# LeiXu84/fireFoam-dev

Measured on AMD Instinct MI355X. Metric: PIMPLE outer-iterations/sec on 64M-cell hex mesh; pEqn SpMV GB/s vs HBM peak, higher is better.
Workload: dtype f64; 1 GPU; synthetic 400^3 hex box (64000000 cells), buoyant plume + 5-species EDC-shaped source, PIMPLE 1/2/0: rhoEqn + UEqn + YEEqn(4 Yi + h) + 2 pEqn per step; cells=64000000, faces=191520000, parallelism=1 GPU, transport_solvers=PBiCGStab+DILU

## Files before the change

### firefoam-dev_amd/binding.py

```python
import ctypes as C
import os
import re
import subprocess

import numpy as np

_HERE = os.path.dirname(os.path.abspath(__file__))
_ROOT = os.path.dirname(_HERE)
_SO = os.path.join(_HERE, "lib", "libffm.so")
_HDR = os.path.join(_ROOT, "include", "ffm.h")

SOLVERS = {"PCG": 0, "PBiCGStab": 1, "PBiCG": 2, "diagonal": 3, "smoothSolver": 4}
PRECONDS = {"none": 0, "DIC": 1, "DILU": 2, "GaussSeidel": 3, "symGaussSeidel": 4, "diagonal": 5}


class FfmError(RuntimeError):
    pass


class Perf(C.Structure):
    _fields_ = [("initialResidual", C.c_double), ("finalResidual", C.c_double),
                ("nIterations", C.c_int), ("converged", C.c_int), ("singular", C.c_int)]

    def as_dict(self):
# ... 65 lines not shown
        "ffm_ldu_set_coeffs_d": ([vp, dp, dp, dp], C.c_int),
        "ffm_ldu_n_native_faces": ([vp], C.c_int),
        "ffm_ldu_get_face_map": ([vp, ip], C.c_int),
        "ffm_ldu_set_coeffs_native_d": ([vp, dp, dp, dp], C.c_int),
        "ffm_ldu_bind_coeffs_native_d": ([vp, dp, dp, dp, C.c_int], C.c_int),
        "ffm_ldu_set_interfaces": ([vp, C.c_int, ip, C.POINTER(ip), C.POINTER(hp), C.POINTER(hp), ip], C.c_int),
        "ffm_ldu_set_global_cells": ([vp, C.c_long], C.c_int),
        "ffm_spmv": ([vp, dp, dp], C.c_int),
        "ffm_tmul": ([vp, dp, dp], C.c_int),
        "ffm_sumA": ([vp, dp], C.c_int),
        "ffm_residual": ([vp, dp, dp, dp], C.c_int),
        "ffm_precond_setup": ([vp, C.c_int, dp], C.c_int),
        "ffm_precond_apply": ([vp, C.c_int, C.c_int, dp, dp], C.c_int),
        "ffm_precond_setup_multi": ([vp, C.c_int, C.c_int, C.POINTER(C.c_void_p), C.POINTER(C.c_void_p)], C.c_int),
        "ffm_ldu_tile_reach": ([vp, C.POINTER(C.c_int), C.POINTER(C.c_int), C.POINTER(C.c_int)], C.c_int),
        "ffm_gs_smooth": ([vp, C.c_int, C.c_int, dp, dp], C.c_int),
        "ffm_solve_d": ([vp, C.c_int, C.c_int, C.c_double, C.c_double, C.c_int, C.c_int, C.c_int, dp, dp,
                         C.POINTER(Perf)], C.c_int),
        "ffm_solve": ([vp, C.c_int, C.c_int, C.c_double, C.c_double, C.c_int, C.c_int, C.c_int, hp, hp,
                       C.POINTER(Perf)], C.c_int),
        "ffm_solve_multi_d": ([vp, C.c_int, C.c_int, C.c_int, C.c_double, C.c_double, C.c_int, C.c_int, C.POINTER(C.c_void_p), dp, dp,
                               C.POINTER(C.c_void_p), C.POINTER(C.c_void_p), C.POINTER(Perf)], C.c_int),
        "ffm_ldu_unbind_coeffs": ([vp], C.c_int),
        "ffm_ldu_offdiag_epoch": ([vp], C.c_ulong),
        "ffm_ldu_tile_coef_read": ([vp, C.c_int, hp], C.c_int),
        "ffm_ldu_tile_gathers": ([vp], C.c_long),
        "ffm_debug_pool_poison": ([vp, C.c_int], C.c_int),
        "ffm_bench_spmv": ([vp, dp, dp, C.c_int, hp], C.c_int),
        "ffm_bench_precond": ([vp, C.c_int, dp, dp, C.c_int, hp], C.c_int),
        "ffm_debug_set_sweep_ticket": ([vp, C.c_uint], C.c_int),
# ... 80 lines not shown
                                           + [C.POINTER(C.c_void_p)] * 16, C.c_int),
        "ffm_fvm_scalar_transport_multi_w": ([vp, C.c_int, dp, C.c_double, dp, dp, dp, dp, dp, dp] + [C.POINTER(C.c_void_p)] * 12, C.c_int),
        "ffm_fvm_scalar_transport_multi_ws": ([vp, C.c_int, dp, C.c_double, dp, dp, dp, dp, dp, dp] + [C.POINTER(C.c_void_p)] * 5 + [hp]
                                              + [C.POINTER(C.c_void_p)] * 7, C.c_int),
        "ffm_fvm_scalar_transport_multi_ws_direct": ([vp, C.c_int, dp, C.c_double, dp, dp, dp, dp, dp, dp] + [C.POINTER(C.c_void_p)] * 5 + [hp]
                                                     + [C.POINTER(C.c_void_p)] * 7, C.c_int),
        "ffm_fv_multivariate_weights": ([vp, C.c_int, C.POINTER(C.c_int), C.c_double, C.c_double, C.c_double, dp] + [C.POINTER(C.c_void_p)] * 4 + [dp], C.c_int),
        "ffm_fvm_lust_source3": ([vp, C.c_double, dp, dp] + [C.POINTER(C.c_void_p)] * 5, C.c_int),
        "ffm_pc_phig": ([vp, dp, dp, dp, dp], C.c_int),
        "ffm_ue_buoyancy_flux": ([vp, dp, dp, dp, dp], C.c_int),
        "ffm_pc_phiHbyA": ([vp, dp, dp, dp, dp, dp, dp, dp, dp], C.c_int),
        "ffm_pc_flux": ([vp, dp, dp, dp, dp, dp, dp, dp, dp, dp], C.c_int),
        "ffm_pc_face_fluxes": ([vp] + [dp] * 10, C.c_int),
        "ffm_pc_finish": ([vp, C.c_double, C.c_double] + [dp] * 9 + [C.POINTER(vp)] + [dp] * 4 + [C.POINTER(vp)] + [dp] * 4, C.c_int),
        "ffm_ue_buoyancy_source3": ([vp, dp, dp, dp, dp, C.POINTER(vp), C.POINTER(vp), dp, C.POINTER(vp), C.POINTER(vp), C.POINTER(vp)], C.c_int),
        "ffm_fvm_transport_scheme": ([vp, C.c_double, dp, dp, C.c_int, dp, C.c_int, dp, dp, dp], C.c_int),
        "ffm_fvm_transport_scheme_direct": ([vp, C.c_double, dp, dp, C.c_int, dp, C.c_int, dp, dp, dp], C.c_int),
        "ffm_fvc_div_dev2T_gradU": ([vp, C.POINTER(vp), dp, dp, C.POINTER(vp), C.POINTER(vp), C.POINTER(vp)], C.c_int),
        "ffm_les_keqn_G": ([vp, C.POINTER(vp), dp, dp], C.c_int),
        "ffm_fvm_HbyA3": ([vp, dp, dp, C.POINTER(vp), C.POINTER(vp), C.POINTER(vp), C.POINTER(vp), dp, C.POINTER(vp)], C.c_int),
        "ffm_fvc_flux_rho": ([vp, dp, dp, dp, dp, dp], C.c_int),
        "ffm_fvm_pressure_eqn": ([vp, C.c_double] + [dp] * 6 + [C.c_double] + [dp] * 9, C.c_int),
        "ffm_fvm_pressure_eqn_direct": ([vp, C.c_double] + [dp] * 6 + [C.c_double] + [dp] * 9, C.c_int),
        "ffm_fvc_ddt_corr": ([vp, C.c_double] + [dp] * 6, C.c_int),
        "ffm_fvc_rho_eqn": ([vp, C.c_double] + [dp] * 4, C.c_int),
        "ffm_fvc_div_phiK_terms": ([vp, C.c_int] + [C.c_double] * 4 + [dp] * 14, C.c_int),
        "ffm_fvdom_ray_assemble_d": ([vp, hp] + [C.c_double] * 3 + [dp] * 9, C.c_int),
        "ffm_fvdom_wall_coeffs_d": ([vp, C.c_int, C.c_int, hp, hp, C.c_double] + [dp] * 8, C.c_int),
        "ffm_fvdom_sum_rays_d": ([vp, C.c_int, dp, dp], C.c_int),
        "ffm_mesh_nboundary": ([vp], C.c_int),
# ... 476 lines not shown

    def reciprocalD_multi(self, preconditioner, diags):
        self.ctx._ready()
        n = len(diags)
        out = [self.ctx.empty(self.nCells) for _ in range(n)]
        arr = lambda ts: (C.c_void_p * n)(*[t.data_ptr() for t in ts])
        _check(lib().ffm_precond_setup_multi(self.h, PRECONDS[preconditioner], n, arr(diags), arr(out)), "ffm_precond_setup_multi")
        self.ctx.sync()
        return out

    def tile_reach(self):
        r, a, b = C.c_int(), C.c_int(), C.c_int()
        _check(lib().ffm_ldu_tile_reach(self.h, C.byref(r), C.byref(a), C.byref(b)), "ffm_ldu_tile_reach")
        return r.value, a.value, b.value

    def precondition(self, preconditioner, rA, transpose=False):
        self.ctx._ready()
        w = self.ctx.empty(self.nCells)
        _check(lib().ffm_precond_apply(self.h, PRECONDS[preconditioner], 1 if transpose else 0,
                                       C.c_void_p(rA.data_ptr()), C.c_void_p(w.data_ptr())), "ffm_precond_apply")
        self.ctx.sync()
        return w

    def smooth(self, psi, source, nSweeps=1, smoother="symGaussSeidel"):
        self.ctx._ready()
        psi = psi.clone()
        self.ctx._ready()
        _check(lib().ffm_gs_smooth(self.h, 1 if smoother == "symGaussSeidel" else 0, nSweeps,
                                   C.c_void_p(psi.data_ptr()), C.c_void_p(source.data_ptr())), "ffm_gs_smooth")
        self.ctx.sync()
# ... 471 lines not shown
```

### firefoam-dev_amd/csrc/ffm_device.hpp

```cpp
#pragma once
#include <hip/hip_runtime.h>
#include "ffm_internal.hpp"

static inline int sgrid(long n) { long g = (n + 255) / 256; return (int)std::max(1L, std::min(g, (long)RED_BLOCKS)); }

__device__ __forceinline__ double wave_sum(double v)
{
#pragma unroll
    for (int o = 32; o > 0; o >>= 1) v += __shfl_down(v, o, 64);
    return v;
}
__device__ __forceinline__ double wave_min(double v)
{
#pragma unroll
    for (int o = 32; o > 0; o >>= 1) v = fmin(v, __shfl_down(v, o, 64));
    return v;
}
__device__ __forceinline__ double wave_max(double v)
{
#pragma unroll
    for (int o = 32; o > 0; o >>= 1) v = fmax(v, __shfl_down(v, o, 64));
    return v;
}

// ... 115 lines not shown
__device__ __forceinline__ void load_lower(const LduView &v, int c, RowEnt<W> &R, int s0 = 0)
{
    const int sl = c >> 6, lane = c & 63;
    const int lb = lo_base(v, sl) + s0 * 64, lw = lo_width(v, sl) - s0;
    int e[W];
#pragma unroll
    for (int s = 0; s < W; s++) e[s] = (s < lw) ? (NT ? __builtin_nontemporal_load(&v.loEnt[lb + s * 64 + lane]) : v.loEnt[lb + s * 64 + lane]) : -1;
#pragma unroll
    for (int s = 0; s < W; s++) {
        R.on[s] = e[s] >= 0;
        R.nb[s] = R.on[s] ? (e[s] >> v.loShift) : c;
        R.f[s] = R.on[s] ? face_of(v, R.nb[s], (int)__builtin_amdgcn_ubfe((unsigned)e[s], 0u, (unsigned)v.loShift)) : 0;
    }
}

template <int W, bool MASK_GHOST = false, bool NT = false>
__device__ __forceinline__ void load_upper(const LduView &v, int c, RowEnt<W> &R, int s0 = 0)
{
    const int sl = c >> 6, lane = c & 63;
    const int ub = up_base(v, sl) + s0 * 64, uw = up_width(v, sl) - s0;
#pragma unroll
    for (int s = 0; s < W; s++) {
        const int idx = ub + s * 64 + lane;
        const int n = (s < uw) ? (NT ? __builtin_nontemporal_load(&v.upNbr[idx]) : v.upNbr[idx]) : -1;
        R.on[s] = n >= 0 && (!MASK_GHOST || n < v.N);
        R.nb[s] = R.on[s] ? n : c;
        R.f[s] = R.on[s] ? idx : 0;
    }
}

// ... 21 lines not shown
```

### firefoam-dev_amd/csrc/ffm_fused.hip

```cpp
#include "ffm_mesh.hpp"

constexpr int FUSE_MAX = 5;
constexpr int FUSE_MAX_OWN = 4;
#define CHECK_M(m) if (!(m)) { ffm_set_error("null mesh"); return FFM_ERR_ARG; }

struct GradMulti {
    const double *vf[FUSE_MAX], *vb[FUSE_MAX];
    double *gx[FUSE_MAX], *gy[FUSE_MAX], *gz[FUSE_MAX];
};

template <int W, int NF>
__global__ __launch_bounds__(256) void k_grad_multi(MeshView q, GradMulti a)
{
    CELL_SCHED(ci, q) {
        const int c = (int)ci;
        RowEnt<W> L, U; load_lower<W>(q.v, c, L); load_upper<W>(q.v, c, U);
        double wl[W], wu[W], sx[2 * W], sy[2 * W], sz[2 * W];
#pragma unroll
        for (int s = 0; s < W; s++) {
            wl[s] = q.w[L.f[s]]; wu[s] = q.w[U.f[s]];
            sx[s] = q.Sfx[L.f[s]]; sy[s] = q.Sfy[L.f[s]]; sz[s] = q.Sfz[L.f[s]];
            sx[W + s] = q.Sfx[U.f[s]]; sy[W + s] = q.Sfy[U.f[s]]; sz[W + s] = q.Sfz[U.f[s]];
        }
        const double V = q.V[c];
// ... 1009 lines not shown
    if (!ghf || !rho || !p_rgh || !diag || !source || !diagOut || !sourceOut || (m->B && (!t_b || !ic || !bc))) return FFM_ERR_ARG;
    UeBuoyancy a;
    for (int d = 0; d < 3; d++) {
        if (!source[d] || !diagOut[d] || !sourceOut[d] || (m->B && (!ic[d] || !bc[d]))) return FFM_ERR_ARG;
        a.ic[d] = m->B ? ic[d] : nullptr; a.bc[d] = m->B ? bc[d] : nullptr; a.src[d] = source[d]; a.diagOut[d] = diagOut[d]; a.srcOut[d] = sourceOut[d];
    }
    a.ghf = ghf; a.rho = rho; a.prgh = p_rgh; a.tb = t_b; a.diag = diag; a.invT = m->invT; a.bMagSf = m->bMagSf; a.invStride = m->N;
    if (m->A->maxW > 8) return FFM_ERR_UNSUPPORTED;
    if (m->A->maxW <= 3) LAUNCH_CELLS(k_ue_buoyancy_source3<3>, mview(m), a);
    else if (m->A->maxW <= 4) LAUNCH_CELLS(k_ue_buoyancy_source3<4>, mview(m), a);
    else LAUNCH_CELLS(k_ue_buoyancy_source3<8>, mview(m), a);
    FFM_HIP(hipGetLastError());
    return FFM_OK;
}

struct PEqn {
    const double *psi, *psi0, *p0, *rho, *rho0, *gh, *gamma, *phiHbyA, *phiHbyAb, *ic, *bc;
    double *upper, *lower, *diag, *src;
    double rdt, pRef;
    TileCoefOut tile;
};
template <int W, bool TILE = false>
__global__ __launch_bounds__(256, (TILE ? 8 : 1)) void k_p_rgh_eqn(MeshView q, PEqn a)
{
    CELL_SCHED(ci, q) {
        const int c = (int)ci;
        RowEnt<W> L, U; load_lower<W>(q.v, c, L); load_upper<W>(q.v, c, U);
        double dLap = 0.0, acc = 0.0;
        double vl[TILE ? W : 1] = {}, vu[TILE ? W : 1] = {};
#pragma unroll
// ... 298 lines not shown
```

### firefoam-dev_amd/csrc/ffm_plume_step.hip

```cpp
#include "ffm_plume.hpp"

static void bc_update_f(ffm_plume *P, double *f, const double *fStatic)
{ const double *pb = P->phib; forN(P, P->B, [=] __device__(long k) { f[k] = fStatic[k] < 0 ? 1.0 - (pb[k] >= 0 ? 1.0 : 0.0) : fStatic[k]; }); }

static int update_bcs(ffm_plume *P)
{
    for (int c = 0; c < 3; c++) bc_update_f(P, P->fU[c], P->fStaticU[c]);
    bc_update_f(P, P->fS, P->fStaticS);
    bc_update_f(P, P->fH, P->fStaticH);
    return FFM_OK;
}

static int U_boundary(ffm_plume *P)
{
    for (int c = 0; c < 3; c++) FFM_TRY(ffm_bc_values(P->mesh, P->fU[c], P->refU[c], P->zeroB, P->U[c], P->Ub[c]));
    return FFM_OK;
}

static int bc_p_rgh(ffm_plume *P, const double *grad , const double *rhob)
{
    const double *kind = P->kind_d, *pb = P->phib, *phb = P->ph_rgh_b;
    const double *u0 = P->Ub[0], *u1 = P->Ub[1], *u2 = P->Ub[2];
    double *f = P->fP, *ref = P->refP, *g = P->gradP;
    forN(P, P->B, [=] __device__(long k) {
// ... 65 lines not shown
    for (int c = 0; c < 3; c++) {
        FFM_TRY(ffm_fvm_boundary_coeffs(m, P->phib, mub, -1, P->fU[c], P->refU[c], P->zeroB, P->Uic[c], P->Ubc[c]));
        if (ops) FFM_TRY(u_source_ops(P, c));
    }
    if (ops) return FFM_OK;
    const double *uf[3] = {P->U[0], P->U[1], P->U[2]}, *ub[3] = {P->Ub[0], P->Ub[1], P->Ub[2]}, *u0[3] = {P->U0[0], P->U0[1], P->U0[2]};
    double *ggx[3] = {P->gM[0][0], P->gM[1][0], P->gM[2][0]}, *ggy[3] = {P->gM[0][1], P->gM[1][1], P->gM[2][1]}, *ggz[3] = {P->gM[0][2], P->gM[1][2], P->gM[2][2]};
    FFM_TRY(ffm_fvc_grad_multi(m, 3, uf, ub, ggx, ggy, ggz));
    for (int c = 0; c < 3; c++) { FFM_TRY(HX(P, ggx[c])); FFM_TRY(HX(P, ggy[c])); FFM_TRY(HX(P, ggz[c])); }
    return ffm_fvm_lust_source3(m, P->rdt, P->phi, P->rho0, u0, ggx, ggy, ggz, P->Usrc);
}

#define DIRECT_OR(P, direct, plain) \
    do { int rc_ = ((P)->oneBlock && ffm_tile_coef_direct_ok((P)->A)) ? (direct) : FFM_ERR_UNSUPPORTED; \
         if (rc_ == FFM_ERR_UNSUPPORTED) rc_ = (plain); FFM_TRY(rc_); } while (0)

static void les_gradU(ffm_plume *P, const double *g9[9])
{ for (int i = 0; i < 3; i++) for (int j = 0; j < 3; j++) g9[3 * i + j] = P->fused ? P->gM[j][i] : P->lesG[j][i]; }

static int les_rho_nuEff_faces(ffm_plume *P, double *gamCell, bool wantCell, double *rhob, double *gf, double *gb)
{
    ffm_mesh *m = P->mesh;
    const double *rho = P->rho, *nut = P->nut, *nutb = P->nutb;
    zg(P, rhob, rho);
    if (!P->fused || wantCell) forN(P, P->N, [=] __device__(long i) { gamCell[i] = rho[i] * (nut[i] + MU / rho[i]); });
    if (P->fused) return ffm_les_face_diffusivity(m, 0, MU, rho, rhob, nut, nutb, gf, gb);
    FFM_TRY(ffm_fvc_interpolate(m, nullptr, gamCell, gf));
    forN(P, P->B, [=] __device__(long k) { gb[k] = rhob[k] * (nutb[k] + MU / rhob[k]); });
    return FFM_OK;
}
// ... 29 lines not shown
    if (ops) FFM_TRY(ffm_fv_limited_weights(m, 4, 1.0, 0.0, 1.0, P->phi, nullptr, nullptr, nullptr, nullptr, wU));
    double *gam = P->wN[8];
    if (P->turbModel) FFM_TRY(les_rho_nuEff_faces(P, gam, true, P->wB[6], muf, mub));
    else {
        forN(P, P->nNat, [=] __device__(long e) { muf[e] = MU; });
        forN(P, P->B, [=] __device__(long k) { mub[k] = MU; });
    }
    if (ops) FFM_TRY(ffm_fvm_transport(m, P->rdt, P->rho, P->phi, wU, muf, -1, P->Udiag, P->Uupper, P->Ulower));
    else DIRECT_OR(P, ffm_fvm_transport_scheme_direct(m, P->rdt, P->rho, P->phi, 4, muf, -1, P->Udiag, P->Uupper, P->Ulower),
                   ffm_fvm_transport_scheme(m, P->rdt, P->rho, P->phi, 4, muf, -1, P->Udiag, P->Uupper, P->Ulower));
    FFM_TRY(u_buoyancy(P, rec));
    FFM_TRY(u_sources(P, mub));
    if (P->turbModel) FFM_TRY(u_stress_divergence(P, gam, mub));
    const char *nm[3] = {"Ux", "Uy", "Uz"};
    if (ops) { for (int c = 0; c < 3; c++) FFM_TRY(ffm_fvm_add_boundary(m, P->Uic[c], P->Ubc[c], P->Udiag, P->Usrc[c], rec[c], P->UdW[c], P->UsW[c])); }
    else FFM_TRY(ffm_ue_buoyancy_source3(m, P->ghf, P->rho, P->p_rgh, P->wB[5], P->Uic, P->Ubc, P->Udiag, P->Usrc, P->UdW, P->UsW));
    FFM_TRY(solve_named_multi(P, 3, nm, 1e-6, P->UdW, P->Uupper, P->Ulower, P->U, P->UsW));
    for (int c = 0; c < 3; c++) FFM_TRY(HX(P, P->U[c]));
    double *K = P->K; const double *U0 = P->U[0], *U1 = P->U[1], *U2 = P->U[2];
    forN(P, N, [=] __device__(long i) { K[i] = 0.5 * ((U0[i] * U0[i] + U1[i] * U1[i]) + U2[i] * U2[i]); });
    return FFM_OK;
}

static void standin_combustion(ffm_plume *P)
{
    double *af = P->alphaEff_f, *afb = P->alphaEff_b, *wFuel = P->wFuel, *Qdot = P->Qdot, *Yt = P->Yt;
    if (!P->turbModel) {
        forN(P, P->nNat, [=] __device__(long e) { af[e] = 0.5 * (MU / PR) + (1.0 - 0.5) * (MU / PR); });
        forN(P, P->B, [=] __device__(long k) { afb[k] = MU / PR; });
    }
    const double *rho = P->rho, *fuel = P->Y[2], *o2 = P->Y[0];
// ... 376 lines not shown
                                        P->ic[0], P->bc[0], P->upper, nullptr, P->dWork, P->sWork));
    FFM_TRY(solve_named(P, "p_rgh", FFM_PCG, FFM_DIC, 1e-6, final ? 0.0 : 0.01, P->dWork, P->upper, nullptr, P->p_rgh, P->sWork));
    return HX(P, P->p_rgh);
}

static int pc_flux_U(ffm_plume *P, const PCorr &w)
{
    ffm_mesh *m = P->mesh; const int N = P->N; const double rdt = P->rdt; const bool ops = !P->fused;
    double *t = P->wF[5], *tb = P->wB[6];
    double *phi = P->phi, *phib = P->phib; const double *phiHbyA = w.phiHbyA, *fl = w.fl, *phig = w.phig, *rhorAUf = w.rhorAUf;
    const double *phiHbyAb = w.phiHbyAb, *flb = w.flb, *rhorAUfb = w.rhorAUfb;
    const double *lower = ops ? P->lower : P->upper;
    FFM_TRY(ffm_fvm_flux(m, P->upper, lower, P->ic[0], P->bc[0], P->p_rgh, ops ? w.fl : nullptr, w.flb));
    if (!ops && P->oneBlock) {
        forN(P, P->B, [=] __device__(long k) { phib[k] = phiHbyAb[k] + flb[k]; tb[k] = flb[k] / rhorAUfb[k]; });
        return ffm_pc_finish(m, rdt, PREF, P->upper, lower, P->p_rgh, phiHbyA, phig, rhorAUf, phib, tb, w.rAU, w.HbyA, P->gh, P->p0, P->rho0,
                             phi, P->U, P->K, P->p, P->dpdt, P->rho);
    }
    if (ops) forN(P, P->nNat, [=] __device__(long e) { phi[e] = phiHbyA[e] + fl[e]; t[e] = rhorAUf[e] != 0.0 ? (fl[e] + phig[e]) / rhorAUf[e] : 0.0; });
    else FFM_TRY(ffm_pc_flux(m, P->upper, lower, P->p_rgh, phiHbyA, phig, rhorAUf, w.fl, phi, t));
    forN(P, P->B, [=] __device__(long k) { phib[k] = phiHbyAb[k] + flb[k]; tb[k] = flb[k] / rhorAUfb[k]; });
    FFM_TRY(ffm_fvc_reconstruct(m, t, tb, w.rec[0], w.rec[1], w.rec[2]));
    const double *rAU = w.rAU, *rx = w.rec[0], *ry = w.rec[1], *rz = w.rec[2], *h0 = w.HbyA[0], *h1 = w.HbyA[1], *h2 = w.HbyA[2];
    double *U0 = P->U[0], *U1 = P->U[1], *U2 = P->U[2], *K = P->K, *dpdt = P->dpdt, *p = P->p;
    const double *rho = P->rho, *p_rgh = P->p_rgh, *gh = P->gh, *p0 = P->p0;
    forN(P, P->nOwn, [=] __device__(long i) {
        const double a = h0[i] + rAU[i] * rx[i], b = h1[i] + rAU[i] * ry[i], c = h2[i] + rAU[i] * rz[i];
        U0[i] = a; U1[i] = b; U2[i] = c;
    });
    FFM_TRY(HX(P, U0)); FFM_TRY(HX(P, U1)); FFM_TRY(HX(P, U2));
    forN(P, N, [=] __device__(long i) { p[i] = p_rgh[i] + rho[i] * gh[i] + PREF; });
    FFM_TRY(rho_eqn(P));
// ... 120 lines not shown
```

### firefoam-dev_amd/csrc/ffm_tile.hip

```cpp
#include "ffm_internal.hpp"
#include "ffm_device.hpp"
#include <algorithm>
#include <atomic>
#include <climits>

constexpr int T_RING = 4096;
constexpr int T_ENT = 256;
constexpr int T_THREADS = 256;
constexpr int T_W = FFM_TILE_W;
constexpr int T_PF = 8;
constexpr int T_PM = 3;
constexpr int T_XMAX = 64;
constexpr int T_RINGD = T_RING - 2 * T_ENT;
constexpr unsigned T_SPIN_LIMIT = 1u << 22;
constexpr unsigned T_NONE = 0xFFFFu;
constexpr int T_LDS = T_RING + 2 * T_XMAX + 1;
constexpr unsigned long long T_SENT = 0x7FF4DEADBEEFCAFEull;
static_assert(T_LDS < (int)T_NONE && T_ENT <= 256, "neighbour codes are LDS slots");
static_assert(T_PM >= 2 && T_PM < T_PF, "read-ahead distances");

struct TileDir {
    int nEnt = 0, nPub = 0;
    int *grpEnt = nullptr;
    int4 *rec = nullptr;
    int *extSrc = nullptr;
    unsigned short *code = nullptr;
    int *src = nullptr;
    double *coefU = nullptr, *coefL = nullptr;
    unsigned long epochU = ~0ul, epochL = ~0ul;
    int reach = 0;
    double *mail = nullptr;
};

struct ffm_tile_plan {
    bool usable = false;
    int G = 0;
    TileDir f, b;
// ... 82 lines not shown
        int seen = reach.load();
        while (far > seen && !reach.compare_exchange_weak(seen, far)) {}
    });
    D.reach = reach;
    if (tooMany) { ok = false; return FFM_OK; }
    std::vector<unsigned short> code((size_t)4 * nOwn, (unsigned short)T_NONE);
    std::vector<int> grpEnt(G + 1, 0), mailIdx(nOwn, -1);
    std::vector<int4> rec;
    int nPub = 0;
    auto extRefs = [&](int c) { int n = 0; for (int k = 0; k < W; k++) { const int nb = nbr[(size_t)W * c + k]; if (nb >= 0 && isExt(c, nb)) n++; } return n; };
    for (int g = 0; g < G; g++) {
        const int gs = grpCell[g], ge = grpCell[g + 1];
        int prevLevel = -1;
        auto close = [&](int c0, int c1, int nExt) {
            if (lvl[c0] < prevLevel) ok = false;
            prevLevel = lvl[c0];
            int slot = 0;
            for (int c = c0; c < c1; c++) if (exposed[c]) { code[(size_t)4 * c + 3] = (unsigned short)slot; mailIdx[c] = nPub + slot; slot++; }
            rec.push_back(make_int4(c0, (c1 - c0) | (nExt << 16), nPub, 0));
            nPub += slot;
        };
        if (fwd) {
            for (int c = gs; c < ge;) {
                int e = c, nx = 0;
                while (e < ge && lvl[e] == lvl[c] && e - c < T_ENT) { const int x = extRefs(e); if (e > c && nx + x > T_XMAX) break; nx += x; e++; }
                close(c, e, nx); c = e;
            }
        } else {
            for (int c = ge; c > gs;) {
                int e = c, nx = 0;
// ... 573 lines not shown
    hipLaunchKernelGGL(k_tile_fill, dim3(g), dim3(256), 0, A->ctx->stream, n, (unsigned long long *)p, T_SENT, A->sweepTicket);
}

bool ffm_tile_multi_fits(const ffm_ldu *A, int n)
{
    if (n < 1 || n > FFM_TILE_MAXSYS || !ffm_tile_usable(A)) return false;
    return n <= 4 || std::max(A->tile->f.reach, A->tile->b.reach) <= TM_RING5 - 2 * T_ENT;
}
extern "C" int ffm_ldu_tile_reach(const ffm_ldu *A, int *reach, int *limit, int *limit5)
{
    if (!A || !reach || !limit || !limit5) return FFM_ERR_ARG;
    if (!ffm_tile_usable(A)) { ffm_set_error("ffm_ldu_tile_reach: the matrix has no tile plan"); return FFM_ERR_UNSUPPORTED; }
    *reach = std::max(A->tile->f.reach, A->tile->b.reach); *limit = T_RINGD; *limit5 = TM_RING5 - 2 * T_ENT;
    return FFM_OK;
}
static int tile_mail(ffm_ldu *A, int n, bool fwdOnly, double **mail)
{
    ffm_tile_plan *T = A->tile;
    if (n > 1 && !T->mailMulti) FFM_HIP(hipMalloc((void **)&T->mailMulti, sizeof(double) * (size_t)FFM_TILE_MAXSYS * (size_t)T->nMail));
    *mail = (n == 1) ? T->mailAll : T->mailMulti;
    tile_fill(A, *mail, (n == 1 && fwdOnly) ? (long)T->f.nPub + 1 : (long)n * T->nMail);
    return FFM_OK;
}
template <int MODE, int NF, int R = T_RING, bool FUSE = false>
static void tile_launch(ffm_ldu *A, const TileDir &d, double *mail, const double *ca, const double *cb, const double *const *dg, const double *const *r,
                        double *const *w, double *aux = nullptr, const double *scal = nullptr, double *partials = nullptr)
{
    ffm_tile_plan *T = A->tile;
    TileSys<NF> m;
    for (int i = 0; i < NF; i++) { m.dg[i] = dg[i]; m.r[i] = r ? r[i] : nullptr; m.w[i] = w[i]; m.mail[i] = mail + (size_t)i * T->nMail + (d.mail - T->mailAll); }
// ... 357 lines not shown
```

### include/ffm.h

```cpp
#ifndef FFM_H
#define FFM_H

#include <stddef.h>
#include <stdint.h>

#ifdef __cplusplus
extern "C" {
#endif

typedef struct ffm_ctx ffm_ctx;
typedef struct ffm_ldu ffm_ldu;

typedef enum ffm_status {
    FFM_OK = 0,
    FFM_ERR_ARG = -1,
    FFM_ERR_ADDR = -2,
    FFM_ERR_HIP = -3,
    FFM_ERR_NODEVICE = -4,
    FFM_ERR_UNSUPPORTED = -5,
    FFM_ERR_COMM = -6
} ffm_status;

typedef enum ffm_solver {
    FFM_PCG = 0, FFM_PBICGSTAB = 1, FFM_PBICG = 2, FFM_DIAGONAL = 3, FFM_SMOOTH = 4,
// ... 88 lines not shown
                           const double *const *bouCoeffs,
                           const double *const *intCoeffs,
                           const int *neighbRank);
int ffm_ldu_set_global_cells(ffm_ldu *ldu, long globalCells);
int ffm_ldu_set_exchange_tags(ffm_ldu *ldu, int kind, int n, const int *tags);

int ffm_spmv(ffm_ldu *ldu, const double *x_d, double *y_d);
int ffm_tmul(ffm_ldu *ldu, const double *x_d, double *y_d);
int ffm_sumA(ffm_ldu *ldu, double *s_d);
int ffm_residual(ffm_ldu *ldu, const double *x_d, const double *b_d, double *r_d);
int ffm_precond_setup(ffm_ldu *ldu, int precond, double *rD_out_d );
int ffm_precond_apply(ffm_ldu *ldu, int precond, int transpose,
                      const double *r_d, double *w_d);
int ffm_precond_setup_multi(ffm_ldu *ldu, int precond, int nSys, const double *const *diag_d, double *const *rD_out_d);
int ffm_ldu_tile_reach(const ffm_ldu *ldu, int *reach, int *limit, int *limit5);
int ffm_gs_smooth(ffm_ldu *ldu, int symmetric_sweep, int nSweeps, double *psi_d,
                  const double *b_d);

int ffm_solve_d(ffm_ldu *ldu, int solver, int precond, double tolerance,
                double relTol, int minIter, int maxIter, int nSweeps,
                double *psi_d, const double *source_d, ffm_perf *out);
int ffm_solve(ffm_ldu *ldu, int solver, int precond, double tolerance,
              double relTol, int minIter, int maxIter, int nSweeps,
              double *psi, const double *source, ffm_perf *out);
int ffm_solve_multi_d(ffm_ldu *ldu, int nSys, int solver, int precond, double tolerance, double relTol, int minIter, int maxIter,
                      const double *const *diag_d, const double *upper_d, const double *lower_d, double *const *psi_d,
                      const double *const *source_d, ffm_perf *out );

int ffm_bench_spmv(ffm_ldu *ldu, const double *x_d, double *y_d, int reps,
                   double *avg_ms);
// ... 81 lines not shown
int ffm_pc_phig(ffm_mesh *m, const double *rhorAUf, const double *ghf, const double *rho, double *phig);
int ffm_pc_phiHbyA(ffm_mesh *m, const double *rho, const double *vx, const double *vy, const double *vz, const double *rhorAUf,
                   const double *ddtCorr, const double *phig, double *phiHbyA);
int ffm_pc_flux(ffm_mesh *m, const double *upper, const double *lower, const double *psi, const double *phiHbyA, const double *phig,
                const double *rhorAUf, double *flux_f, double *phi_f, double *t_f);
int ffm_ue_buoyancy_flux(ffm_mesh *m, const double *ghf, const double *rho, const double *p_rgh, double *t_f);
int ffm_pc_face_fluxes(ffm_mesh *m, const double *rhorAU, const double *ghf, const double *rho, const double *vx, const double *vy,
                       const double *vz, const double *ddtCorr, double *rhorAUf, double *phig, double *phiHbyA);
int ffm_pc_finish(ffm_mesh *m, double rDeltaT, double pRef, const double *upper, const double *lower, const double *p_rgh,
                  const double *phiHbyA, const double *phig, const double *rhorAUf, const double *phi_b, const double *t_b,
                  const double *rAU, const double *const *HbyA, const double *gh, const double *p0, const double *rho0,
                  double *phi_f, double *const *U, double *K, double *p, double *dpdt, double *rho);
int ffm_ue_buoyancy_source3(ffm_mesh *m, const double *ghf, const double *rho, const double *p_rgh, const double *t_b,
                            const double *const *internalCoeffs, const double *const *boundaryCoeffs, const double *diag,
                            const double *const *source, double *const *diagOut, double *const *sourceOut);
int ffm_fvc_flux_rho(ffm_mesh *m, const double *rho, const double *vx, const double *vy, const double *vz, double *out_f);
int ffm_fvc_ddt_corr(ffm_mesh *m, double rDeltaT, const double *rho0, const double *vx0, const double *vy0, const double *vz0,
                     const double *phi0_f, double *out_f);
int ffm_fvm_rAU(ffm_mesh *m, int nCmpt, const double *diag, const double *ic0, const double *ic1, const double *ic2,
                const double *psi, const double *p, double *rho, double *rAU, double *rhorAU);
int ffm_fvc_rho_eqn(ffm_mesh *m, double rDeltaT, const double *phi_f, const double *phi_b, const double *rho0, double *rho);
int ffm_fvc_div_phiK_terms(ffm_mesh *m, int scheme, double k, double lo, double hi, double rDeltaT, const double *phi_f,
                           const double *phi_b, const double *K, const double *K_b, const double *gx, const double *gy,
                           const double *gz, const double *rho, const double *rho0, const double *K0, const double *dpdt,
                           double *divK, double *ddtK, double *negDpdt);
int ffm_fvm_flux(ffm_mesh *m, const double *upper, const double *lower, const double *internalCoeffs,
                 const double *boundaryCoeffs, const double *psi, double *out_f, double *out_b);

int ffm_fvc_grad_multi(ffm_mesh *m, int nf, const double *const *vf, const double *const *vb, double *const *gx,
                       double *const *gy, double *const *gz);
// ... 210 lines not shown
```

Before: 3.236 outer-iterations/s.

## Add face-window tiled kernels for pressure finish and buoyancy source

Adds a k_face_window kernel that walks the tile plan's segments of cell groups in order and keeps each group's per-face upper contributions in shared memory. The next group can then read its lower-face values from that buffer instead of recomputing them, which roughly halves face work and gathers for the pEqn finish and UEqn buoyancy source. Both paths are used only for meshes with at least 32M cells, and fall back to the existing kernels when tiling is unsupported. The cost is heavy shared-memory use per block, which limits occupancy, plus extra syncthreads per group. Lower faces whose neighbour is outside the previous group are still recomputed.

```diff
diff --git a/firefoam-dev_amd/binding.py b/firefoam-dev_amd/binding.py
--- a/firefoam-dev_amd/binding.py
+++ b/firefoam-dev_amd/binding.py
@@ -103,6 +103,7 @@
         "ffm_precond_apply": ([vp, C.c_int, C.c_int, dp, dp], C.c_int),
         "ffm_precond_setup_multi": ([vp, C.c_int, C.c_int, C.POINTER(C.c_void_p), C.POINTER(C.c_void_p)], C.c_int),
         "ffm_ldu_tile_reach": ([vp, C.POINTER(C.c_int), C.POINTER(C.c_int), C.POINTER(C.c_int)], C.c_int),
+        "ffm_ldu_tile_entries": ([vp, C.POINTER(C.c_int), C.POINTER(C.c_int), C.POINTER(C.c_int)], C.c_int),
         "ffm_gs_smooth": ([vp, C.c_int, C.c_int, dp, dp], C.c_int),
         "ffm_solve_d": ([vp, C.c_int, C.c_int, C.c_double, C.c_double, C.c_int, C.c_int, C.c_int, dp, dp,
                          C.POINTER(Perf)], C.c_int),
@@ -213,6 +214,8 @@
         "ffm_pc_face_fluxes": ([vp] + [dp] * 10, C.c_int),
         "ffm_pc_finish": ([vp, C.c_double, C.c_double] + [dp] * 9 + [C.POINTER(vp)] + [dp] * 4 + [C.POINTER(vp)] + [dp] * 4, C.c_int),
         "ffm_ue_buoyancy_source3": ([vp, dp, dp, dp, dp, C.POINTER(vp), C.POINTER(vp), dp, C.POINTER(vp), C.POINTER(vp), C.POINTER(vp)], C.c_int),
+        "ffm_pc_finish_tiled": ([vp, C.c_double, C.c_double] + [dp] * 9 + [C.POINTER(vp)] + [dp] * 4 + [C.POINTER(vp)] + [dp] * 4, C.c_int),
+        "ffm_ue_buoyancy_source3_tiled": ([vp, dp, dp, dp, dp, C.POINTER(vp), C.POINTER(vp), dp, C.POINTER(vp), C.POINTER(vp), C.POINTER(vp)], C.c_int),
         "ffm_fvm_transport_scheme": ([vp, C.c_double, dp, dp, C.c_int, dp, C.c_int, dp, dp, dp], C.c_int),
         "ffm_fvm_transport_scheme_direct": ([vp, C.c_double, dp, dp, C.c_int, dp, C.c_int, dp, dp, dp], C.c_int),
         "ffm_fvc_div_dev2T_gradU": ([vp, C.POINTER(vp), dp, dp, C.POINTER(vp), C.POINTER(vp), C.POINTER(vp)], C.c_int),
@@ -719,6 +722,11 @@
         _check(lib().ffm_ldu_tile_reach(self.h, C.byref(r), C.byref(a), C.byref(b)), "ffm_ldu_tile_reach")
         return r.value, a.value, b.value
 
+    def tile_entries(self):
+        g, e, k = C.c_int(), C.c_int(), C.c_int()
+        _check(lib().ffm_ldu_tile_entries(self.h, C.byref(g), C.byref(e), C.byref(k)), "ffm_ldu_tile_entries")
+        return g.value, e.value, k.value
+
     def precondition(self, preconditioner, rA, transpose=False):
         self.ctx._ready()
         w = self.ctx.empty(self.nCells)
diff --git a/firefoam-dev_amd/csrc/ffm_device.hpp b/firefoam-dev_amd/csrc/ffm_device.hpp
--- a/firefoam-dev_amd/csrc/ffm_device.hpp
+++ b/firefoam-dev_amd/csrc/ffm_device.hpp
@@ -153,6 +153,26 @@
     }
 }
 
+template <int W, bool NT = false>
+__device__ __forceinline__ void fetch_lower(const LduView &v, int c, int (&e)[W])
+{
+    const int sl = c >> 6, lane = c & 63;
+    const int lb = lo_base(v, sl), lw = lo_width(v, sl);
+#pragma unroll
+    for (int s = 0; s < W; s++) e[s] = (s < lw) ? (NT ? __builtin_nontemporal_load(&v.loEnt[lb + s * 64 + lane]) : v.loEnt[lb + s * 64 + lane]) : -1;
+}
+template <int W>
+__device__ __forceinline__ void decode_lower(const LduView &v, int c, const int (&e)[W], RowEnt<W> &R, int (&slot)[W])
+{
+#pragma unroll
+    for (int s = 0; s < W; s++) {
+        R.on[s] = e[s] >= 0;
+        R.nb[s] = R.on[s] ? (e[s] >> v.loShift) : c;
+        slot[s] = R.on[s] ? (int)__builtin_amdgcn_ubfe((unsigned)e[s], 0u, (unsigned)v.loShift) : 0;
+        R.f[s] = R.on[s] ? face_of(v, R.nb[s], slot[s]) : 0;
+    }
+}
+
 template <int W, bool MASK_GHOST = false, bool NT = false>
 __device__ __forceinline__ void load_upper(const LduView &v, int c, RowEnt<W> &R, int s0 = 0)
 {
diff --git a/firefoam-dev_amd/csrc/ffm_fused.hip b/firefoam-dev_amd/csrc/ffm_fused.hip
--- a/firefoam-dev_amd/csrc/ffm_fused.hip
+++ b/firefoam-dev_amd/csrc/ffm_fused.hip
@@ -1047,6 +1047,187 @@
     return FFM_OK;
 }
 
+constexpr int FW_ENT = 256;
+template <class PASS, int NBUF>
+__global__ __launch_bounds__(256) void k_face_window(MeshView q, PASS a, const int4 *__restrict__ seg, const int4 *__restrict__ rec)
+{
+    constexpr int NV = PASS::NV, W = FFM_TILE_W;
+    __shared__ double buf[NBUF][W * NV * FW_ENT];
+    const int4 sg = seg[blockIdx.x];
+    const int gBeg = sg.x, ea = sg.y, eb = sg.z;
+    const int t = threadIdx.x;
+    int pc0 = 0, pcnt = 0;
+    int4 R = rec[max(ea - 1, gBeg)];
+    RowEnt<W> U; int le[W];
+    { const int c = R.x + (t < (R.y & 0xFFFF) ? t : 0); load_upper<W>(q.v, c, U); fetch_lower<W>(q.v, c, le); }
+    for (int ee = max(ea - 1, gBeg); ee < eb; ee++) {
+        const int c0 = R.x, cnt = R.y & 0xFFFF;
+        const int4 Rn = rec[ee + 1 < eb ? ee + 1 : ee];
+        RowEnt<W> Un; int len[W];
+        { const int cn = Rn.x + (t < (Rn.y & 0xFFFF) ? t : 0); load_upper<W>(q.v, cn, Un); fetch_lower<W>(q.v, cn, len); }
+        double *mine = buf[NBUF == 2 ? (ee & 1) : 0]; const double *prev = buf[NBUF == 2 ? ((ee & 1) ^ 1) : 0];
+        const bool act = t < cnt, fin = act && ee >= ea;
+        const int c = c0 + (act ? t : 0);
+        const typename PASS::Cell own = a.cell(c);
+        RowEnt<W> L; int slot[W]; decode_lower<W>(q.v, c, le, L, slot);
+        double up[W][NV], lo[W][NV];
+#pragma unroll
+        for (int s = 0; s < W; s++) a.face(q, U.f[s], own, a.cell(U.nb[s]), up[s]);
+        if (ee >= ea) {
+#pragma unroll
+            for (int s = 0; s < W; s++) {
+                const int d = L.nb[s] - pc0;
+                if (L.on[s] && (unsigned)d < (unsigned)pcnt) {
+#pragma unroll
+                    for (int k = 0; k < NV; k++) lo[s][k] = prev[(slot[s] * NV + k) * FW_ENT + d];
+                } else if (L.on[s]) a.face(q, L.f[s], a.cell(L.nb[s]), own, lo[s]);
+                else {
+#pragma unroll
+                    for (int k = 0; k < NV; k++) lo[s][k] = 0.0;
+                }
+            }
+        }
+        if (NBUF == 1) __syncthreads();
+        if (act) {
+#pragma unroll
+            for (int s = 0; s < W; s++)
+#pragma unroll
+                for (int k = 0; k < NV; k++) mine[(s * NV + k) * FW_ENT + t] = up[s][k];
+        }
+        if (fin) a.finish(q, c, own, L, U, lo, up);
+        pc0 = c0; pcnt = cnt; R = Rn; U = Un;
+#pragma unroll
+        for (int s = 0; s < W; s++) le[s] = len[s];
+        __syncthreads();
+    }
+}
+
+struct PcFinishTile : PcFinish {
+    static constexpr int NV = 4;
+    struct Cell { double p; };
+    __device__ __forceinline__ Cell cell(int c) const { return {prgh[c]}; }
+    __device__ __forceinline__ void face(const MeshView &q, int e, const Cell &o, const Cell &n, double (&out)[NV]) const
+    {
+        const double raf = rhorAUf[e];
+        const double f = upper[e] * n.p - lower[e] * o.p;
+        out[0] = phiHbyA[e] + f;
+        const double tv = raf != 0.0 ? (f + phig[e]) / raf : 0.0, mg = q.magSf[e];
+        out[1] = q.Sfx[e] / mg * tv; out[2] = q.Sfy[e] / mg * tv; out[3] = q.Sfz[e] / mg * tv;
+    }
+    __device__ __forceinline__ void finish(const MeshView &q, int c, const Cell &own, const RowEnt<FFM_TILE_W> &L, const RowEnt<FFM_TILE_W> &U,
+                                           const double (&lo)[FFM_TILE_W][NV], const double (&up)[FFM_TILE_W][NV]) const
+    {
+        constexpr int W = FFM_TILE_W;
+        const PcFinish &a = *this; const long N = a.invStride;
+        const double P = own.p;
+        RecSum v = {0.0, 0.0, 0.0};
+        double acc = 0.0, pe[W];
+#pragma unroll
+        for (int s = 0; s < W; s++) if (L.on[s]) { acc = acc - lo[s][0]; v.x += lo[s][1]; v.y += lo[s][2]; v.z += lo[s][3]; }
+#pragma unroll
+        for (int s = 0; s < W; s++) {
+            pe[s] = 0.0;
+            if (U.on[s]) { pe[s] = up[s][0]; acc += pe[s]; v.x += up[s][1]; v.y += up[s][2]; v.z += up[s][3]; }
+        }
+        const int j = q.cellB[c];
+        if (j >= 0) for (int t = q.bcStart[j]; t < q.bcStart[j + 1]; t++) {
+            const int k = q.bcItem[t]; const double b = a.tb[k], mg = a.bMagSf[k];
+            v.x += q.bSfx[k] / mg * b; v.y += q.bSfy[k] / mg * b; v.z += q.bSfz[k] / mg * b;
+            acc += a.phib[k];
+        }
+        const double xx = a.invT[c], xy = a.invT[N + c], xz = a.invT[2 * N + c], yy = a.invT[3 * N + c], yz = a.invT[4 * N + c], zz = a.invT[5 * N + c];
+        const double rx = xx * v.x + xy * v.y + xz * v.z, ry = xy * v.x + yy * v.y + yz * v.z, rz = xz * v.x + yz * v.y + zz * v.z;
+        const double r = a.rAU[c];
+        const double u0 = a.H[0][c] + r * rx, u1 = a.H[1][c] + r * ry, u2 = a.H[2][c] + r * rz;
+        a.U[0][c] = u0; a.U[1][c] = u1; a.U[2][c] = u2;
+        a.K[c] = 0.5 * ((u0 * u0 + u1 * u1) + u2 * u2);
+        const double pp = P + a.rho[c] * a.gh[c] + a.pRef;
+        a.p[c] = pp; a.dpdt[c] = a.rdt * (pp - a.p0[c]);
+        const double V = q.V[c], div = acc / V;
+        a.rho[c] = (a.rdt * a.rho0[c] * V - V * div) / (a.rdt * V);
+        const int sl = c >> 6, ub = up_base(q.v, sl) + (c & 63), uw = up_width(q.v, sl);
+#pragma unroll
+        for (int s = 0; s < W; s++) if (s < uw) a.phi[ub + s * 64] = pe[s];
+    }
+};
+struct UeBuoyancyTile : UeBuoyancy {
+    static constexpr int NV = 3;
+    struct Cell { double r, p; };
+    __device__ __forceinline__ Cell cell(int c) const { return {rho[c], prgh[c]}; }
+    __device__ __forceinline__ void face(const MeshView &q, int e, const Cell &o, const Cell &n, double (&out)[NV]) const
+    {
+        const double sgr = q.delta[e] * (n.r - o.r), sgp = q.delta[e] * (n.p - o.p);
+        const double mg = q.magSf[e], tv = (-ghf[e] * sgr - sgp) * mg;
+        out[0] = q.Sfx[e] / mg * tv; out[1] = q.Sfy[e] / mg * tv; out[2] = q.Sfz[e] / mg * tv;
+    }
+    __device__ __forceinline__ void finish(const MeshView &q, int c, const Cell &, const RowEnt<FFM_TILE_W> &L, const RowEnt<FFM_TILE_W> &U,
+                                           const double (&lo)[FFM_TILE_W][NV], const double (&up)[FFM_TILE_W][NV]) const
+    {
+        constexpr int W = FFM_TILE_W;
+        const UeBuoyancy &a = *this; const long N = a.invStride;
+        RecSum v = {0.0, 0.0, 0.0};
+#pragma unroll
+        for (int s = 0; s < W; s++) if (L.on[s]) { v.x += lo[s][0]; v.y += lo[s][1]; v.z += lo[s][2]; }
+#pragma unroll
+        for (int s = 0; s < W; s++) if (U.on[s]) { v.x += up[s][0]; v.y += up[s][1]; v.z += up[s][2]; }
+        double bd[3] = {0.0, 0.0, 0.0}, bs[3] = {0.0, 0.0, 0.0};
+        const double d0 = a.diag[c];
+#pragma unroll
+        for (int d = 0; d < 3; d++) { bd[d] = d0; bs[d] = a.src[d][c]; }
+        const int j = q.cellB[c];
+        if (j >= 0) for (int t = q.bcStart[j]; t < q.bcStart[j + 1]; t++) {
+            const int k = q.bcItem[t]; const double b = a.tb[k], mg = a.bMagSf[k];
+            v.x += q.bSfx[k] / mg * b; v.y += q.bSfy[k] / mg * b; v.z += q.bSfz[k] / mg * b;
+#pragma unroll
+            for (int d = 0; d < 3; d++) { bd[d] += a.ic[d][k]; bs[d] += a.bc[d][k]; }
+        }
+        const double xx = a.invT[c], xy = a.invT[N + c], xz = a.invT[2 * N + c], yy = a.invT[3 * N + c], yz = a.invT[4 * N + c], zz = a.invT[5 * N + c];
+        const double rec[3] = {xx * v.x + xy * v.y + xz * v.z, xy * v.x + yy * v.y + yz * v.z, xz * v.x + yz * v.y + zz * v.z};
+        const double V = q.V[c];
+#pragma unroll
+        for (int d = 0; d < 3; d++) { a.diagOut[d][c] = bd[d]; a.srcOut[d][c] = bs[d] + V * rec[d]; }
+    }
+};
+static bool face_window_segments(ffm_mesh *m, FfmFvSegs *sg) { return m->A->maxW <= FFM_TILE_W && ffm_tile_fv_segments(m->A, MVT_RUN, sg); }
+
+extern "C" int ffm_pc_finish_tiled(ffm_mesh *m, double rDeltaT, double pRef, const double *upper, const double *lower, const double *p_rgh,
+                                   const double *phiHbyA, const double *phig, const double *rhorAUf, const double *phi_b, const double *t_b,
+                                   const double *rAU, const double *const *HbyA, const double *gh, const double *p0, const double *rho0,
+                                   double *phi_f, double *const *U, double *K, double *p, double *dpdt, double *rho)
+{
+    CHECK_M(m);
+    if (!upper || !lower || !p_rgh || !phiHbyA || !phig || !rhorAUf || !rAU || !HbyA || !gh || !p0 || !rho0 || !phi_f || !U || !K || !p ||
+        !dpdt || !rho || rho == rho0 || (m->B && (!phi_b || !t_b))) return FFM_ERR_ARG;
+    PcFinishTile a;
+    for (int d = 0; d < 3; d++) { if (!HbyA[d] || !U[d]) return FFM_ERR_ARG; a.H[d] = HbyA[d]; a.U[d] = U[d]; }
+    a.upper = upper; a.lower = lower; a.prgh = p_rgh; a.phiHbyA = phiHbyA; a.phig = phig; a.rhorAUf = rhorAUf; a.phib = phi_b; a.tb = t_b;
+    a.rAU = rAU; a.gh = gh; a.p0 = p0; a.rho0 = rho0; a.invT = m->invT; a.bMagSf = m->bMagSf;
+    a.phi = phi_f; a.K = K; a.p = p; a.dpdt = dpdt; a.rho = rho; a.rdt = rDeltaT; a.pRef = pRef; a.invStride = m->N;
+    FfmFvSegs sg;
+    if (!face_window_segments(m, &sg)) return FFM_ERR_UNSUPPORTED;
+    hipLaunchKernelGGL((k_face_window<PcFinishTile, 1>), dim3(sg.nSeg), dim3(256), 0, m->ctx->stream, mview(m), a, sg.seg, sg.rec);
+    FFM_HIP(hipGetLastError());
+    return FFM_OK;
+}
+extern "C" int ffm_ue_buoyancy_source3_tiled(ffm_mesh *m, const double *ghf, const double *rho, const double *p_rgh, const double *t_b,
+                                             const double *const *ic, const double *const *bc, const double *diag, const double *const *source,
+                                             double *const *diagOut, double *const *sourceOut)
+{
+    CHECK_M(m);
+    if (!ghf || !rho || !p_rgh || !diag || !source || !diagOut || !sourceOut || (m->B && (!t_b || !ic || !bc))) return FFM_ERR_ARG;
+    UeBuoyancyTile a;
+    for (int d = 0; d < 3; d++) {
+        if (!source[d] || !diagOut[d] || !sourceOut[d] || (m->B && (!ic[d] || !bc[d]))) return FFM_ERR_ARG;
+        a.ic[d] = m->B ? ic[d] : nullptr; a.bc[d] = m->B ? bc[d] : nullptr; a.src[d] = source[d]; a.diagOut[d] = diagOut[d]; a.srcOut[d] = sourceOut[d];
+    }
+    a.ghf = ghf; a.rho = rho; a.prgh = p_rgh; a.tb = t_b; a.diag = diag; a.invT = m->invT; a.bMagSf = m->bMagSf; a.invStride = m->N;
+    FfmFvSegs sg;
+    if (!face_window_segments(m, &sg)) return FFM_ERR_UNSUPPORTED;
+    hipLaunchKernelGGL((k_face_window<UeBuoyancyTile, 2>), dim3(sg.nSeg), dim3(256), 0, m->ctx->stream, mview(m), a, sg.seg, sg.rec);
+    FFM_HIP(hipGetLastError());
+    return FFM_OK;
+}
+
 struct PEqn {
     const double *psi, *psi0, *p0, *rho, *rho0, *gh, *gamma, *phiHbyA, *phiHbyAb, *ic, *bc;
     double *upper, *lower, *diag, *src;
diff --git a/firefoam-dev_amd/csrc/ffm_plume_step.hip b/firefoam-dev_amd/csrc/ffm_plume_step.hip
--- a/firefoam-dev_amd/csrc/ffm_plume_step.hip
+++ b/firefoam-dev_amd/csrc/ffm_plume_step.hip
@@ -103,6 +103,10 @@
 #define DIRECT_OR(P, direct, plain) \
     do { int rc_ = ((P)->oneBlock && ffm_tile_coef_direct_ok((P)->A)) ? (direct) : FFM_ERR_UNSUPPORTED; \
          if (rc_ == FFM_ERR_UNSUPPORTED) rc_ = (plain); FFM_TRY(rc_); } while (0)
+constexpr long FACE_WINDOW_MIN_CELLS = 32L << 20;
+#define TILED_OR(P, tiled, plain) \
+    do { int rc_ = ((P)->nOwn >= FACE_WINDOW_MIN_CELLS) ? (tiled) : FFM_ERR_UNSUPPORTED; \
+         if (rc_ == FFM_ERR_UNSUPPORTED) rc_ = (plain); FFM_TRY(rc_); } while (0)
 
 static void les_gradU(ffm_plume *P, const double *g9[9])
 { for (int i = 0; i < 3; i++) for (int j = 0; j < 3; j++) g9[3 * i + j] = P->fused ? P->gM[j][i] : P->lesG[j][i]; }
@@ -162,7 +166,8 @@
     if (P->turbModel) FFM_TRY(u_stress_divergence(P, gam, mub));
     const char *nm[3] = {"Ux", "Uy", "Uz"};
     if (ops) { for (int c = 0; c < 3; c++) FFM_TRY(ffm_fvm_add_boundary(m, P->Uic[c], P->Ubc[c], P->Udiag, P->Usrc[c], rec[c], P->UdW[c], P->UsW[c])); }
-    else FFM_TRY(ffm_ue_buoyancy_source3(m, P->ghf, P->rho, P->p_rgh, P->wB[5], P->Uic, P->Ubc, P->Udiag, P->Usrc, P->UdW, P->UsW));
+    else TILED_OR(P, ffm_ue_buoyancy_source3_tiled(m, P->ghf, P->rho, P->p_rgh, P->wB[5], P->Uic, P->Ubc, P->Udiag, P->Usrc, P->UdW, P->UsW),
+                  ffm_ue_buoyancy_source3(m, P->ghf, P->rho, P->p_rgh, P->wB[5], P->Uic, P->Ubc, P->Udiag, P->Usrc, P->UdW, P->UsW));
     FFM_TRY(solve_named_multi(P, 3, nm, 1e-6, P->UdW, P->Uupper, P->Ulower, P->U, P->UsW));
     for (int c = 0; c < 3; c++) FFM_TRY(HX(P, P->U[c]));
     double *K = P->K; const double *U0 = P->U[0], *U1 = P->U[1], *U2 = P->U[2];
@@ -569,8 +574,11 @@
     FFM_TRY(ffm_fvm_flux(m, P->upper, lower, P->ic[0], P->bc[0], P->p_rgh, ops ? w.fl : nullptr, w.flb));
     if (!ops && P->oneBlock) {
         forN(P, P->B, [=] __device__(long k) { phib[k] = phiHbyAb[k] + flb[k]; tb[k] = flb[k] / rhorAUfb[k]; });
-        return ffm_pc_finish(m, rdt, PREF, P->upper, lower, P->p_rgh, phiHbyA, phig, rhorAUf, phib, tb, w.rAU, w.HbyA, P->gh, P->p0, P->rho0,
-                             phi, P->U, P->K, P->p, P->dpdt, P->rho);
+        TILED_OR(P, ffm_pc_finish_tiled(m, rdt, PREF, P->upper, lower, P->p_rgh, phiHbyA, phig, rhorAUf, phib, tb, w.rAU, w.HbyA, P->gh, P->p0, P->rho0,
+                                     phi, P->U, P->K, P->p, P->dpdt, P->rho),
+                 ffm_pc_finish(m, rdt, PREF, P->upper, lower, P->p_rgh, phiHbyA, phig, rhorAUf, phib, tb, w.rAU, w.HbyA, P->gh, P->p0, P->rho0,
+                               phi, P->U, P->K, P->p, P->dpdt, P->rho));
+        return FFM_OK;
     }
     if (ops) forN(P, P->nNat, [=] __device__(long e) { phi[e] = phiHbyA[e] + fl[e]; t[e] = rhorAUf[e] != 0.0 ? (fl[e] + phig[e]) / rhorAUf[e] : 0.0; });
     else FFM_TRY(ffm_pc_flux(m, P->upper, lower, P->p_rgh, phiHbyA, phig, rhorAUf, w.fl, phi, t));
diff --git a/firefoam-dev_amd/csrc/ffm_tile.hip b/firefoam-dev_amd/csrc/ffm_tile.hip
--- a/firefoam-dev_amd/csrc/ffm_tile.hip
+++ b/firefoam-dev_amd/csrc/ffm_tile.hip
@@ -21,6 +21,7 @@
 
 struct TileDir {
     int nEnt = 0, nPub = 0;
+    int nCont = 0;
     int *grpEnt = nullptr;
     int4 *rec = nullptr;
     int *extSrc = nullptr;
@@ -133,6 +134,7 @@
         int prevLevel = -1;
         auto close = [&](int c0, int c1, int nExt) {
             if (lvl[c0] < prevLevel) ok = false;
+            if (lvl[c0] == prevLevel) D.nCont++;
             prevLevel = lvl[c0];
             int slot = 0;
             for (int c = c0; c < c1; c++) if (exposed[c]) { code[(size_t)4 * c + 3] = (unsigned short)slot; mailIdx[c] = nPub + slot; slot++; }
@@ -736,6 +738,13 @@
     *reach = std::max(A->tile->f.reach, A->tile->b.reach); *limit = T_RINGD; *limit5 = TM_RING5 - 2 * T_ENT;
     return FFM_OK;
 }
+extern "C" int ffm_ldu_tile_entries(const ffm_ldu *A, int *groups, int *entries, int *continued)
+{
+    if (!A || !groups || !entries || !continued) return FFM_ERR_ARG;
+    if (!ffm_tile_usable(A)) { ffm_set_error("ffm_ldu_tile_entries: the matrix has no tile plan"); return FFM_ERR_UNSUPPORTED; }
+    *groups = A->tile->G; *entries = A->tile->f.nEnt; *continued = A->tile->f.nCont;
+    return FFM_OK;
+}
 static int tile_mail(ffm_ldu *A, int n, bool fwdOnly, double **mail)
 {
     ffm_tile_plan *T = A->tile;
diff --git a/include/ffm.h b/include/ffm.h
--- a/include/ffm.h
+++ b/include/ffm.h
@@ -126,6 +126,7 @@
                       const double *r_d, double *w_d);
 int ffm_precond_setup_multi(ffm_ldu *ldu, int precond, int nSys, const double *const *diag_d, double *const *rD_out_d);
 int ffm_ldu_tile_reach(const ffm_ldu *ldu, int *reach, int *limit, int *limit5);
+int ffm_ldu_tile_entries(const ffm_ldu *ldu, int *groups, int *entries, int *continued);
 int ffm_gs_smooth(ffm_ldu *ldu, int symmetric_sweep, int nSweeps, double *psi_d,
                   const double *b_d);
 
@@ -237,6 +238,13 @@
 int ffm_ue_buoyancy_source3(ffm_mesh *m, const double *ghf, const double *rho, const double *p_rgh, const double *t_b,
                             const double *const *internalCoeffs, const double *const *boundaryCoeffs, const double *diag,
                             const double *const *source, double *const *diagOut, double *const *sourceOut);
+int ffm_pc_finish_tiled(ffm_mesh *m, double rDeltaT, double pRef, const double *upper, const double *lower, const double *p_rgh,
+                        const double *phiHbyA, const double *phig, const double *rhorAUf, const double *phi_b, const double *t_b,
+                        const double *rAU, const double *const *HbyA, const double *gh, const double *p0, const double *rho0,
+                        double *phi_f, double *const *U, double *K, double *p, double *dpdt, double *rho);
+int ffm_ue_buoyancy_source3_tiled(ffm_mesh *m, const double *ghf, const double *rho, const double *p_rgh, const double *t_b,
+                                  const double *const *internalCoeffs, const double *const *boundaryCoeffs, const double *diag,
+                                  const double *const *source, double *const *diagOut, double *const *sourceOut);
 int ffm_fvc_flux_rho(ffm_mesh *m, const double *rho, const double *vx, const double *vy, const double *vz, double *out_f);
 int ffm_fvc_ddt_corr(ffm_mesh *m, double rDeltaT, const double *rho0, const double *vx0, const double *vy0, const double *vz0,
                      const double *phi0_f, double *out_f);
```

After: 3.228 outer-iterations/s (median of 2 runs). Within noise of the previous version (-0.3%).
